# gMedAI-Lab/GAViKO

Measured on AMD Instinct MI355X. Metric: MRI volumes/sec (fwd+bwd) ViT-B/16 gaviko, 120x160x160, higher is better.
Workload: dtype bf16

## Files before the change

### gaviko_amd/csrc/common.hpp

```cpp
#pragma once
#include <hip/hip_runtime.h>
#include <functional>
#include <stdint.h>

namespace gvk {

typedef __bf16 bf16;
typedef __attribute__((ext_vector_type(8))) __bf16 bf16x8;
typedef __attribute__((ext_vector_type(4))) __bf16 bf16x4;
typedef __attribute__((ext_vector_type(2))) __bf16 bf16x2;
typedef __attribute__((ext_vector_type(4))) float f32x4;
typedef __attribute__((ext_vector_type(2))) float f32x2;
typedef __attribute__((ext_vector_type(16))) float f32x16;
typedef __attribute__((ext_vector_type(4))) short s16x4;
typedef __attribute__((ext_vector_type(4))) unsigned int u32x4;
typedef __attribute__((ext_vector_type(2))) unsigned int u32x2;

#define GVK_LDS __attribute__((address_space(3)))
#define GVK_GLOBAL __attribute__((address_space(1)))

constexpr int kWave = 64;

__device__ __forceinline__ int lane_id() { return threadIdx.x & 63; }
__device__ __forceinline__ int wave_id() { return __builtin_amdgcn_readfirstlane(threadIdx.x >> 6); }

__device__ __forceinline__ float wave_sum(float v) {
#pragma unroll
  for (int o = 32; o > 0; o >>= 1) v += __shfl_xor(v, o, 64);
  return v;
}
__device__ __forceinline__ float wave_max(float v) {
#pragma unroll
  for (int o = 32; o > 0; o >>= 1) v = fmaxf(v, __shfl_xor(v, o, 64));
  return v;
}

__device__ __forceinline__ void xcd_group_block(int bid, int nblk, int ngrp, int& grp, int& blk) {
  const int per = ngrp >> 3, main = per * 8 * nblk;
  if (bid < main) {
    const int xcd = bid & 7, j = bid >> 3;
    grp = (j / nblk) * 8 + xcd;
    blk = j - (j / nblk) * nblk;
  } else {
    const int r = bid - main;
    grp = per * 8 + r / nblk;
    blk = r - (r / nblk) * nblk;
  }
}

__device__ __forceinline__ void glds16(const void* gsrc, void* lds_wave_base) {
  __builtin_amdgcn_global_load_lds((const GVK_GLOBAL void*)gsrc, (GVK_LDS void*)lds_wave_base, 16, 0, 0);
}

__device__ __forceinline__ bf16x4 lds_read_tr16(const void* p) {
  s16x4 v = __builtin_amdgcn_ds_read_tr16_b64_v4i16((GVK_LDS s16x4*)p);
  return __builtin_bit_cast(bf16x4, v);
}

__device__ __forceinline__ float as_poly(float t) {
  float p = __builtin_fmaf(t, 1.061405429f, -1.453152027f);
  p = __builtin_fmaf(t, p, 1.421413741f);
  p = __builtin_fmaf(t, p, -0.284496736f);
  p = __builtin_fmaf(t, p, 0.254829592f);
  return t * p;
}
__device__ __forceinline__ float erf_fast(float x) {
  const float ax = fabsf(x);
  const float t = __builtin_amdgcn_rcpf(__builtin_fmaf(0.3275911f, ax, 1.0f));
  const float e = __builtin_amdgcn_exp2f(ax * ax * -1.44269504088896340736f);
  const float r = __builtin_fmaf(-as_poly(t), e, 1.0f);
  return copysignf(r, x);
}
__device__ __forceinline__ float gelu_erf(float x) { return 0.5f * x * (1.0f + erff(x * 0.70710678118654752440f)); }
__device__ __forceinline__ float gelu_erf_grad(float x) {
  return 0.5f * (1.0f + erff(x * 0.70710678118654752440f)) + x * 0.39894228040143267794f * __expf(-0.5f * x * x);
}
__device__ __forceinline__ float gelu_fast(float x) {
  const float h = 0.5f * x;
  return __builtin_fmaf(h, erf_fast(x * 0.70710678118654752440f), h);
}
__device__ __forceinline__ float gelu_fast_grad(float x) {
  const float ax = fabsf(x) * 0.70710678118654752440f;
  const float t = __builtin_amdgcn_rcpf(__builtin_fmaf(0.3275911f, ax, 1.0f));
  const float e = __builtin_amdgcn_exp2f(x * x * -0.72134752044448170368f);
  const float erfv = copysignf(__builtin_fmaf(-as_poly(t), e, 1.0f), x);
  return __builtin_fmaf(x * 0.39894228040143267794f, e, __builtin_fmaf(0.5f, erfv, 0.5f));
}
__device__ __forceinline__ void gelu_fast_both(float x, float& y, float& dy) {
  const float z = x * 0.70710678118654752440f, ax = fabsf(z);
  const float t = __builtin_amdgcn_rcpf(__builtin_fmaf(0.3275911f, ax, 1.0f));
  const float e = __builtin_amdgcn_exp2f(ax * ax * -1.44269504088896340736f);
  const float erfv = copysignf(__builtin_fmaf(-as_poly(t), e, 1.0f), z);
  const float h = 0.5f * x;
  y = __builtin_fmaf(h, erfv, h);
  dy = __builtin_fmaf(x * 0.39894228040143267794f, e, __builtin_fmaf(0.5f, erfv, 0.5f));
}
__device__ __forceinline__ float sigmoidf_(float x) { return 1.0f / (1.0f + __expf(-x)); }
__device__ __forceinline__ float quick_gelu(float x) { return x * sigmoidf_(1.702f * x); }
__device__ __forceinline__ float quick_gelu_grad(float x) {
  float s = sigmoidf_(1.702f * x);
  return s + 1.702f * x * s * (1.0f - s);
}

}

#include <stdlib.h>
namespace gvk {
#ifdef GVK_DIAG
inline const char* diag_env(const char* name) { return getenv(name); }
#else
inline const char* diag_env(const char*) { return nullptr; }
#endif
}

extern "C" const char* gvk_last_error(void);
namespace gvk {
int set_error(int code, const char* fmt, ...);

bool plan_recording();
void plan_push(std::function<void()>&& node);
void plan_push_launch(hipStream_t stream, std::function<void()>&& node);

template <typename... KArgs, typename... Args>
inline void launch(void (*kernel)(KArgs...), dim3 grid, dim3 block, unsigned lds, hipStream_t stream, Args... args) {
  if (plan_recording())
    plan_push_launch(stream, [=]() { hipLaunchKernelGGL(kernel, grid, block, lds, stream, static_cast<KArgs>(args)...); });
  hipLaunchKernelGGL(kernel, grid, block, lds, stream, static_cast<KArgs>(args)...);
}
#define GVK_LAUNCH(kernel, grid, block, lds, stream, ...) ::gvk::launch(kernel, grid, block, lds, stream, __VA_ARGS__)

int check_launch(const char* what);
}

#define GVK_REQUIRE(cond, ...)                                  \
  do {                                                          \
    if (!(cond)) return gvk::set_error(-2, __VA_ARGS__);        \
  } while (0)
```

### gaviko_amd/csrc/runtime.hip

```cpp
#include "common.hpp"
#include "../../include/gaviko_hip.h"
#include <cstdarg>
#include <cstdio>
#include <cstdlib>
#include <cstring>
#include <memory>
#include <mutex>
#include <vector>

namespace gvk {
static thread_local char g_err[512] = "";

int set_error(int code, const char* fmt, ...) {
  va_list ap;
  va_start(ap, fmt);
  vsnprintf(g_err, sizeof(g_err), fmt, ap);
  va_end(ap);
  return code;
}

int check_launch(const char* what) {
  hipError_t e = hipGetLastError();
  if (e != hipSuccess) return set_error(-1, "%s: launch failed: %s", what, hipGetErrorString(e));
  return 0;
}

struct Plan {
  std::vector<std::function<void()>> nodes;
  std::vector<hipEvent_t> events;
  ~Plan() {
    for (hipEvent_t e : events) (void)hipEventDestroy(e);
  }
};
static thread_local Plan* g_rec = nullptr;
static std::mutex g_plans_mu;
static std::vector<std::unique_ptr<Plan>> g_plans;

static bool g_plan_timing = false;
bool plan_recording() { return g_rec != nullptr; }
void plan_push(std::function<void()>&& node) { g_rec->nodes.push_back(std::move(node)); }

#ifdef GVK_DIAG
__global__ void nop_kernel() {}
static std::vector<hipStream_t> g_nop_streams;
void plan_push_launch(hipStream_t stream, std::function<void()>&& node) {
  for (hipStream_t s : g_nop_streams)
    if (s == stream) {
      g_rec->nodes.push_back([=]() { hipLaunchKernelGGL(nop_kernel, dim3(1), dim3(64), 0, stream); });
      return;
    }
  g_rec->nodes.push_back(std::move(node));
}
#else
void plan_push_launch(hipStream_t, std::function<void()>&& node) { g_rec->nodes.push_back(std::move(node)); }
#endif

__global__ void seed_advance_kernel(unsigned long long* seed, unsigned long long inc) { seed[0] += inc; }
__global__ __launch_bounds__(256) void fill_u32_kernel(unsigned* p, unsigned v, long n4, long n) {
  const long stride = (long)gridDim.x * 256;
  for (long i = (long)blockIdx.x * 256 + threadIdx.x; i < n4; i += stride) ((uint4*)p)[i] = uint4{v, v, v, v};
  for (long i = 4 * n4 + (long)blockIdx.x * 256 + threadIdx.x; i < n; i += stride) p[i] = v;
}
__global__ __launch_bounds__(256) void copy_u32_kernel(unsigned* dst, const unsigned* src, long n4, long n) {
  const long stride = (long)gridDim.x * 256;
  for (long i = (long)blockIdx.x * 256 + threadIdx.x; i < n4; i += stride) ((uint4*)dst)[i] = ((const uint4*)src)[i];
  for (long i = 4 * n4 + (long)blockIdx.x * 256 + threadIdx.x; i < n; i += stride) dst[i] = src[i];
}
__global__ void scale_kernel(float* x, float alpha, long n) {
  const long i = (long)blockIdx.x * blockDim.x + threadIdx.x;
  if (i < n) x[i] *= alpha;
}
}

#ifdef GVK_DIAG
extern "C" int gvk_plan_nop_stream(void* stream) {
  gvk::g_nop_streams.push_back((hipStream_t)stream);
  return 0;
}
extern "C" int gvk_plan_nop_clear(void) {
  gvk::g_nop_streams.clear();
  return 0;
}
#endif

extern "C" int gvk_plan_begin(void) {
  using namespace gvk;
  GVK_REQUIRE(g_rec == nullptr, "gvk_plan_begin: a plan is already being recorded on this thread");
  g_rec = new Plan();
  return 0;
}

extern "C" int gvk_plan_abort(void) {
  delete gvk::g_rec;
  gvk::g_rec = nullptr;
  return 0;
}

extern "C" int gvk_plan_end(void) {
  using namespace gvk;
  GVK_REQUIRE(g_rec != nullptr, "gvk_plan_end: no plan is being recorded");
  std::lock_guard<std::mutex> lk(g_plans_mu);
  g_plans.emplace_back(g_rec);
  g_rec = nullptr;
  return (int)g_plans.size() - 1;
}

extern "C" int gvk_plan_size(int plan) {
  using namespace gvk;
  std::lock_guard<std::mutex> lk(g_plans_mu);
  GVK_REQUIRE(plan >= 0 && plan < (int)g_plans.size() && g_plans[plan], "gvk_plan_size: no such plan %d", plan);
  return (int)g_plans[plan]->nodes.size();
}

extern "C" int gvk_plan_replay(int plan) {
  using namespace gvk;
  Plan* p = nullptr;
  {
    std::lock_guard<std::mutex> lk(g_plans_mu);
    GVK_REQUIRE(plan >= 0 && plan < (int)g_plans.size() && g_plans[plan], "gvk_plan_replay: no such plan %d", plan);
    p = g_plans[plan].get();
  }
  GVK_REQUIRE(g_rec == nullptr, "gvk_plan_replay: cannot replay while recording");
  for (auto& node : p->nodes) node();
  return check_launch("plan_replay");
}

extern "C" int gvk_plan_free(int plan) {
  using namespace gvk;
  std::lock_guard<std::mutex> lk(g_plans_mu);
  GVK_REQUIRE(plan >= 0 && plan < (int)g_plans.size() && g_plans[plan], "gvk_plan_free: no such plan %d", plan);
  g_plans[plan].reset();
  return 0;
}

extern "C" int gvk_plan_set_timing(int on) {
  gvk::g_plan_timing = on != 0;
  return 0;
}

extern "C" int gvk_plan_event_elapsed(int plan, int e0, int e1, float* ms) {
  using namespace gvk;
  std::lock_guard<std::mutex> lk(g_plans_mu);
  GVK_REQUIRE(plan >= 0 && plan < (int)g_plans.size() && g_plans[plan], "gvk_plan_event_elapsed: no such plan %d", plan);
  Plan* p = g_plans[plan].get();
  GVK_REQUIRE(e0 >= 0 && e1 >= 0 && e0 < (int)p->events.size() && e1 < (int)p->events.size() && ms, "gvk_plan_event_elapsed: bad event ids");
  hipError_t e = hipEventElapsedTime(ms, p->events[e0], p->events[e1]);
  if (e != hipSuccess) return set_error(-1, "hipEventElapsedTime: %s (timing needs GAVIKO_HIP_PLAN_TIMING=1 at record time)", hipGetErrorString(e));
  return 0;
}

static int plan_event_record_impl(void* stream, bool force_sys_fence);
extern "C" int gvk_plan_event_record(void* stream) { return plan_event_record_impl(stream, false); }
extern "C" int gvk_plan_event_record_fenced(void* stream) { return plan_event_record_impl(stream, true); }

static int plan_event_record_impl(void* stream, bool force_sys_fence) {
  using namespace gvk;
  GVK_REQUIRE(g_rec != nullptr, "gvk_plan_event_record: only valid while a plan is being recorded");
  static const bool env_timing = getenv("GAVIKO_HIP_PLAN_TIMING") != nullptr;
  hipEvent_t ev;
  static const bool sys_fence = diag_env("GAVIKO_HIP_EVENT_FENCE") != nullptr;
  const unsigned flags = ((env_timing || g_plan_timing) ? hipEventDefault : hipEventDisableTiming) | ((sys_fence || force_sys_fence) ? 0u : hipEventDisableSystemFence);
  hipError_t e = hipEventCreateWithFlags(&ev, flags);
  if (e != hipSuccess) return set_error(-1, "hipEventCreate: %s", hipGetErrorString(e));
  g_rec->events.push_back(ev);
  hipStream_t s = (hipStream_t)stream;
  g_rec->nodes.push_back([=]() { (void)hipEventRecord(ev, s); });
  e = hipEventRecord(ev, s);
  if (e != hipSuccess) return set_error(-1, "hipEventRecord: %s", hipGetErrorString(e));
  return (int)g_rec->events.size() - 1;
}

extern "C" int gvk_plan_event_stream_wait(int plan, int event, void* stream) {
  using namespace gvk;
  hipEvent_t ev;
  {
    std::lock_guard<std::mutex> lk(g_plans_mu);
    GVK_REQUIRE(plan >= 0 && plan < (int)g_plans.size() && g_plans[plan], "gvk_plan_event_stream_wait: no such plan %d", plan);
    Plan* p = g_plans[plan].get();
    GVK_REQUIRE(event >= 0 && event < (int)p->events.size(), "gvk_plan_event_stream_wait: no such event %d", event);
    ev = p->events[event];
  }
  hipError_t e = hipStreamWaitEvent((hipStream_t)stream, ev, 0);
  if (e != hipSuccess) return set_error(-1, "hipStreamWaitEvent: %s", hipGetErrorString(e));
  return 0;
}

extern "C" int gvk_plan_event_wait(void* stream, int event) {
  using namespace gvk;
  GVK_REQUIRE(g_rec != nullptr, "gvk_plan_event_wait: only valid while a plan is being recorded");
  GVK_REQUIRE(event >= 0 && event < (int)g_rec->events.size(), "gvk_plan_event_wait: no such event %d", event);
  hipEvent_t ev = g_rec->events[event];
  hipStream_t s = (hipStream_t)stream;
  g_rec->nodes.push_back([=]() { (void)hipStreamWaitEvent(s, ev, 0); });
  hipError_t e = hipStreamWaitEvent(s, ev, 0);
  if (e != hipSuccess) return set_error(-1, "hipStreamWaitEvent: %s", hipGetErrorString(e));
  return 0;
}

extern "C" int gvk_memset_async(void* ptr, int value, size_t bytes, void* stream) {
  using namespace gvk;
  GVK_REQUIRE(ptr != nullptr || bytes == 0, "gvk_memset_async: null pointer");
  if (bytes == 0) return 0;
  GVK_REQUIRE(((uintptr_t)ptr & 15) == 0 && bytes % 4 == 0, "gvk_memset_async: pointer must be 16-byte aligned and the size a multiple of 4");
  const unsigned b = (unsigned)value & 0xFFu, v = b | (b << 8) | (b << 16) | (b << 24);
  const long n = (long)(bytes / 4), n4 = n / 4;
  long blocks = (n4 + 255) / 256;
  blocks = blocks < 1 ? 1 : (blocks > 2048 ? 2048 : blocks);
  GVK_LAUNCH(fill_u32_kernel, dim3((unsigned)blocks), dim3(256), 0, (hipStream_t)stream, (unsigned*)ptr, v, n4, n);
  return check_launch("memset_async");
}

extern "C" int gvk_seed_advance(void* seed, uint64_t inc, void* stream) {
  using namespace gvk;
  GVK_REQUIRE(seed != nullptr, "gvk_seed_advance: null pointer");
  GVK_LAUNCH(seed_advance_kernel, dim3(1), dim3(1), 0, (hipStream_t)stream, (unsigned long long*)seed, (unsigned long long)inc);
  return check_launch("seed_advance");
}

extern "C" int gvk_scale_f32(float* x, float alpha, long n, void* stream) {
  using namespace gvk;
  GVK_REQUIRE(x != nullptr && n >= 0, "gvk_scale_f32: bad arguments");
  if (n == 0) return 0;
  GVK_LAUNCH(scale_kernel, dim3((unsigned)((n + 255) / 256)), dim3(256), 0, (hipStream_t)stream, x, alpha, n);
  return check_launch("scale_f32");
}

extern "C" const char* gvk_last_error(void) { return gvk::g_err; }
extern "C" int gvk_abi_version(void) { return 14; }

extern "C" int gvk_device_check(void) {
  int dev = 0;
  hipError_t e = hipGetDevice(&dev);
  if (e != hipSuccess) return gvk::set_error(-1, "hipGetDevice: %s", hipGetErrorString(e));
  hipDeviceProp_t prop;
  e = hipGetDeviceProperties(&prop, dev);
  if (e != hipSuccess) return gvk::set_error(-1, "hipGetDeviceProperties: %s", hipGetErrorString(e));
  if (strncmp(prop.gcnArchName, "gfx950", 6) != 0)
    return gvk::set_error(-4, "libgaviko_hip is built for gfx950 only; device %d is %s", dev, prop.gcnArchName);
  return 950;
}
```

### gaviko_amd/lib.py

```python
from __future__ import annotations

import ctypes as C
import os

import torch

_HERE = os.path.dirname(os.path.abspath(__file__))
if os.environ.get("GPU_MAX_HW_QUEUES") is None:
    os.environ["GPU_MAX_HW_QUEUES"] = "8"
    try:
        import sys as _sys
        _t = _sys.modules.get("torch")
        if _t is not None and _t.cuda.is_initialized():
            import warnings as _w
            _w.warn("gaviko_amd: HIP was initialised before gaviko_amd was imported, so GPU_MAX_HW_QUEUES=8 cannot take effect; the three "
                    "streams of a step may share hardware queues (slower, not wrong).  Import gaviko_amd first or export the variable.")
    except Exception:
        pass

ABI_VERSION = 14
DIAG = os.environ.get("GAVIKO_HIP_DIAG", "0") == "1"
LIB_PATH = os.environ.get("GAVIKO_HIP_LIB") or os.path.join(_HERE, "libgaviko_hip_diag.so" if DIAG else "libgaviko_hip.so")


def diag_env(name: str, default=None):
    return os.environ.get(name, default) if DIAG else default


class GemmDesc(C.Structure):
    _fields_ = [
        ("a", C.c_void_p), ("w", C.c_void_p), ("out0", C.c_void_p), ("out1", C.c_void_p),
        ("bias", C.c_void_p), ("res", C.c_void_p), ("aux", C.c_void_p), ("pos", C.c_void_p), ("seed_ptr", C.c_void_p),
        ("M", C.c_int32), ("N", C.c_int32), ("K", C.c_int32),
        ("lda", C.c_int32), ("ldw", C.c_int32), ("ldo", C.c_int32), ("ldres", C.c_int32), ("ldaux", C.c_int32),
        ("epilogue", C.c_int32), ("rows_in", C.c_int32), ("rows_out", C.c_int32), ("row_off", C.c_int32),
        ("tile", C.c_int32), ("drop_p", C.c_float), ("seed", C.c_uint64),
        ("scale_cols", C.c_int32), ("col_scale", C.c_float),
        ("ln_mean", C.c_void_p), ("ln_rstd", C.c_void_p), ("ln_c1", C.c_void_p), ("stat_part", C.c_void_p), ("stat_pivot", C.c_void_p),
        ("m_panels", C.c_int32), ("m_stride", C.c_int32), ("splitk_ws", C.c_void_p), ("splitk_ws_bytes", C.c_uint64),
        ("ksplit", C.c_int32), ("aux_is_grad", C.c_int32),
    ]


def _struct(name, ptrs, ints, floats=(), u64=(), i64=()):
    fields = [(f, C.c_void_p) for f in ptrs] + [(f, C.c_int32) for f in ints] + [(f, C.c_float) for f in floats] + \
             [(f, C.c_uint64) for f in u64] + [(f, C.c_int64) for f in i64]
    return type(name, (C.Structure,), {"_fields_": fields})


SkinnyDownDesc = _struct("SkinnyDownDesc",
                         ["x", "w", "bias", "ln_gamma", "ln_beta", "mean", "rstd", "z", "y", "w2", "y2", "seed_ptr"],
                         ["M", "C", "L", "L2", "act", "w_layout", "act_in"], ["eps", "drop_p"], ["seed"])
SkinnyUpDesc = _struct("SkinnyUpDesc", ["lat", "w", "bias", "res", "out", "lat_override", "seed_ptr", "ln_x", "ln_mean", "ln_rstd", "ln_gamma", "out_bf16",
                                        "alpha_ptr", "gg_x", "w2", "bias2", "z2", "y2", "lat_b", "w_b",
                                        "nx_w", "nx_bias", "nx_ln_gamma", "nx_ln_beta", "nx_mean", "nx_rstd", "nx_lat", "nx_w2", "nx_y2"],
                       ["M", "C", "L", "T", "P", "w_layout", "accumulate", "L2", "act2", "w2_layout", "nx_L2"], ["drop_p", "drop2_p", "nx_eps"],
                       ["seed", "seed2"])
OuterDesc = _struct("OuterDesc", ["narrow", "wide", "lat_override", "mean", "rstd", "ln_gamma", "ln_beta", "scratch", "out", "colsum", "seed_ptr",
                                  "narrow2", "wide2"],
                    ["M", "C", "L", "T", "P", "transposed", "accumulate", "wide_act", "M2"], ["drop_p"], ["seed"])
WindowAttnDesc = _struct("WindowAttnDesc", ["qkv", "ctx", "lse", "dctx", "delta", "dqkv", "seed_ptr"],
                         ["B", "D", "H", "W", "kd", "kh", "kw", "L"], ["scale", "drop_p"], ["seed"])
GpaDesc = _struct("GpaDesc",
                  ["xl", "ll", "ca0_g", "ca0_b", "ca1_w", "ca1_b", "ca3_w", "ca3_b", "gl0_g", "gl0_b", "gl1_w", "gl1_b",
                   "wgq", "bgq", "wlq", "blq", "imp", "gw", "enh", "prm", "qg", "ql", "cg", "cl", "lse_g", "lse_l",
                   "dcomb", "zx", "zl", "dimp", "dgw_part", "dqg", "dql", "dcg", "dcl", "delta_g", "delta_l", "dprm",
                   "dcls", "gate_partials", "dzx", "dzl", "enh16"],
                  ["B", "T", "N", "P", "L", "ld16", "col16"], ["scale"])
SsfColgradDesc = _struct("SsfColgradDesc", ["dy", "y0", "y1", "pos", "s", "t", "ds", "dt", "scratch"],
                         ["M", "N", "ld_dy", "ld_y", "dy_f32", "y0_f32", "rows_in", "rows_out", "row_off", "y0_cols"], ["y0_mul", "y_mul"])
DvptDesc = _struct("DvptDesc", ["z", "enh", "lse", "dcomb", "gate", "bu", "colsum_dy", "delta", "dz", "dgate"], ["B", "T", "P", "L", "C"], ["scale"])
AdamDesc = _struct("AdamDesc", ["ptr_tab", "blk_tab", "grad", "m", "v", "norm_sq"], ["nblocks"],
                   ["lr", "beta1", "beta2", "eps", "bias_c1", "bias_c2", "max_norm"])
LossDesc = _struct("LossDesc", ["logits", "target", "weights", "loss", "dlogits", "meter"], ["B", "K", "kind", "reduction"], ["gamma", "eps"], i64=["ignore_index"])
DropoutDesc = _struct("DropoutDesc", ["x", "out32", "out16", "seed_ptr"], ["M", "N", "ld", "rows_in", "rows_out", "row_off"], ["drop_p"], ["seed"])
RowProjDesc = _struct("RowProjDesc", ["w", "bias", "y", "z", "y_split"], ["L", "w_layout", "act", "ld_split", "col_split"])
LnBwdDesc = _struct("LnBwdDesc", ["dy", "x", "mean", "rstd", "gamma", "dres", "dx", "dx_bf16", "proj"],
                    ["M", "C", "groups", "rows_per_group", "group_stride", "dy_bf16"])
AttentionDesc = _struct("AttentionDesc", ["qkv", "out", "lse", "dout", "delta", "dqkv", "seed_ptr", "ws"],
                        ["B", "T", "H", "ld_qkv", "ld_out", "f32", "need_rows"], ["scale", "drop_p"], ["seed", "ws_bytes"])
ReduceJob = _struct("ReduceJob", ["a", "b", "out", "a2"], ["M", "J", "L", "accumulate", "M2"])
PgradOuter = _struct("PgradOuter", ["narrow", "wide", "narrow2", "wide2", "lat_override", "mean", "rstd", "out", "colsum",
                                    "aff_w", "aff_gamma", "aff_beta", "aff_dgamma", "aff_dbeta", "aff_dbias"],
                     ["M", "M2", "T", "P", "transposed", "accumulate", "C"], ["drop_p"], ["seed"])
WindowColsumDesc = _struct("WindowColsumDesc", ["qkv", "lse", "w", "out"], ["B", "D", "H", "W", "kd", "kh", "kw", "L"], ["scale"])
GpaMapsDesc = _struct("GpaMapsDesc", ["xl", "ll", "qg", "ql", "lse_g", "lse_l", "imp", "gw", "pg", "pl", "fused"], ["B", "T", "N", "P", "L"])
FeatureTopkDesc = _struct("FeatureTopkDesc", ["q", "g", "exclude", "idx", "score", "scratch"], ["Nq", "Ng", "C", "k", "metric", "nslabs"],
                          i64=["scratch_words"])
HeadDesc = _struct("HeadDesc", ["g", "ln_gamma", "ln_beta", "wh", "bh", "logits", "pooled", "dlogits", "dg", "dwh", "dbh"],
                   ["B", "T", "C", "K", "r0", "R", "accumulate"])

(EPI_STORE_BF16, EPI_BIAS_RES_F32, EPI_BIAS_GELU_BF16, EPI_PATCH_F32, EPI_GELU_BWD_BF16, EPI_STORE_F32, EPI_BIAS_RES_F32_BF16,
 EPI_BIAS_RELU_BF16, EPI_RELU_BWD_BF16) = range(9)

_P, _I, _F, _L = C.c_void_p, C.c_int, C.c_float, C.c_int64
SIGNATURES = {
    "gvk_gemm_nt_bf16": [C.POINTER(GemmDesc), _P],
    "gvk_gemm_nt_f32": [C.POINTER(GemmDesc), _P],
    "gvk_patchify_f32": [_P, _P, _I, _I, _I, _I, _I, _I, _I, _P],
    "gvk_transpose_f32": [_P, _P, _I, _I, _P],
    "gvk_transpose_bf16": [_P, _P, _I, _I, _P],
    "gvk_copy_async": [_P, _P, C.c_size_t, _P],
    "gvk_copy_f32_strided": [_P, _P, _I, _I, _I, _P],
    "gvk_cast_f32_bf16": [_P, _P, _L, _P],
    "gvk_transpose_cast_f32_bf16": [_P, _P, _I, _I, _P],
    "gvk_pack_split_bf16": [_P, _I, _P, _P, _I, _I, _I, _I, _P],
    "gvk_prompt_up_fix": [_P, _P, _P, _P, _I, _I, _I, _I, _I, _P],
    "gvk_layernorm_fwd_fix": [_P, _P, _P, _P, _P, _P, _I, _I, _F, _P, _P, _P, _I, _I, _I, _P],
    "gvk_patchify_bf16": [_P, _P, _I, _I, _I, _I, _I, _I, _I, _P],
    "gvk_layernorm_fwd": [_P, _P, _P, _P, _P, _P, _P, _I, _I, _F, _P],
    "gvk_layernorm_bwd": [C.POINTER(LnBwdDesc), _P],
    "gvk_layernorm_bwd_affine": [_P, _P, _P, _P, _P, _P, _P, _I, _I, _I, _P],
    "gvk_attention_fwd": [C.POINTER(AttentionDesc), _P],
    "gvk_attention_bwd": [C.POINTER(AttentionDesc), _P],
    "gvk_qkv_prescale_bf16": [_P, _I, _I, _I, _F, _P],
    "gvk_prompt_up_fix_stats": [_P, _P, _P, _P, _P, _P, _I, _P, _P, _P, _I, _I, _I, _I, _I, _F, _P],
    "gvk_attention_colsum_bf16": [_P, _P, _P, _I, _P, _I, _I, _I, _I, _I, _I, _P],
    "gvk_rollout_step": [_P, _P, _P, _I, _I, _I, _P],
    "gvk_attention_gradcolsum_bf16": [_P, _P, _P, _I, _P, _I, _P, _I, _I, _I, _I, _I, _I, _P],
    "gvk_relevance_step": [_P, _P, _P, _I, _I, _I, _P],
    "gvk_unpatchify_f32": [_P, _P, _P, _P, _I, _I, _I, _I, _I, _I, _I, _I, _F, _F, _P],
    "gvk_patch_reduce_f32": [_P, _P, _I, _I, _I, _I, _I, _I, _I, _I, _P],
    "gvk_evp_highpass_sign": [_P, _P, _P, _P, _P, _I, _I, _I, _I, _P],
    "gvk_evp_highpass_linear": [_P, _P, _P, _P, _I, _I, _I, _I, _I, _P],
    "gvk_skinny_down": [C.POINTER(SkinnyDownDesc), _P],
    "gvk_skinny_up": [C.POINTER(SkinnyUpDesc), _P],
    "gvk_outer_reduce": [C.POINTER(OuterDesc), _P],
    "gvk_small_wgrad": [_P, _P, _P, _P, _I, _I, _I, _I, _P],
    "gvk_ln_lowrank_affine": [_P, _P, _P, _P, _P, _P, _P, _P, _P, _I, _I, _I, _P],
    "gvk_colsum": [_P, _P, _P, _I, _I, _I, _P],
    "gvk_reduce_batch": [C.POINTER(ReduceJob), _I, _P, _P],
    "gvk_param_grads": [C.POINTER(PgradOuter), _I, C.POINTER(ReduceJob), _I, _P, _L, _P, _I, _P, _I, _I, _P],
    "gvk_window_attn_fwd": [C.POINTER(WindowAttnDesc), _P],
    "gvk_window_attn_bwd": [C.POINTER(WindowAttnDesc), _P],
    "gvk_gpa_fwd": [C.POINTER(GpaDesc), _P],
    "gvk_gpa_bwd": [C.POINTER(GpaDesc), _P],
    "gvk_window_attn_colsum": [C.POINTER(WindowColsumDesc), _P],
    "gvk_gpa_attn_maps": [C.POINTER(GpaMapsDesc), _P],
    "gvk_rows_broadcast": [_P, _P, _P, _I, _I, _I, _I, _I, _P],
    "gvk_rows_batch_sum": [_P, _P, _P, _I, _I, _I, _I, _I, _I, _P],
    "gvk_small_linear_fwd": [_P, _P, _P, _P, _I, _I, _I, _P],
    "gvk_small_linear_bwd": [_P, _P, _P, _P, _P, _P, _I, _I, _I, _I, _P],
    "gvk_vpt_repack_fwd": [_P, _P, _P, _I, _I, _I, _I, _I, _I, _P],
    "gvk_vpt_repack_bwd": [_P, _P, _I, _I, _I, _I, _I, _I, _P],
    "gvk_cast_bf16_f32_strided": [_P, _P, _I, _I, _I, _P],
    "gvk_lora_merge_f32": [_P, _P, _P, _P, _P, _P, _I, _I, _F, _P],
    "gvk_layernorm_fwd_proj": [_P, _P, _P, _P, _P, _P, _I, _I, _F, C.POINTER(RowProjDesc), _P],
    "gvk_layernorm_bwd_up": [_P, _P, _P, _P, _P, _P, _P, _P, _P, _P, _I, _I, _I, _I, _P],
    "gvk_ssf_fold_weight": [_P, _P, _P, _P, _I, _I, _I, _P],
    "gvk_ssf_fold_vec": [_P, _P, _P, _P, _I, _P],
    "gvk_ssf_colgrad": [C.POINTER(SsfColgradDesc), _P],
    "gvk_ssf_ln_grad": [_P, _P, _P, _P, _P, _P, _I, _P],
    "gvk_ssf_head_grad": [_P, _P, _P, _P, _P, _P, _P, _P, _P, _I, _I, _I, _I, _I, _I, _P],
    "gvk_dvpt_fwd": [C.POINTER(DvptDesc), _P],
    "gvk_dvpt_bwd": [C.POINTER(DvptDesc), _P],
    "gvk_scale_dev": [_P, _P, C.c_int64, _P],
    "gvk_evp_highpass": [_P, _P, _P, _P, _I, _I, _I, _I, _P],
    "gvk_pad2d_f32": [_P, _I, _I, _I, _I, _P, _I, _I, _I, _P],
    "gvk_add2d_f32": [_P, _I, _P, _I, _P, _I, _I, _I, _P],
    "gvk_gelu_fwd_f32": [_P, _P, C.c_int64, _P],
    "gvk_gelu_bwd_f32": [_P, _P, _P, C.c_int64, _P],
    "gvk_rows_patch": [_P, _P, _P, _I, _I, _I, _I, _I, _I, _P],
    "gvk_rows_gather": [_P, _P, _I, _I, _I, _I, _I, _P],
    "gvk_sumsq": [_P, C.c_int64, _P, _P, _P],
    "gvk_adam_step": [C.POINTER(AdamDesc), _P],
    "gvk_loss_fwd_bwd": [C.POINTER(LossDesc), _P],
    "gvk_dropout_rows": [C.POINTER(DropoutDesc), _P],
    "gvk_volume_minmax": [_P, _P, _I, _L, _P],
    "gvk_rescale_intensity": [_P, _P, _P, _P, _I, _L, _F, _F, _P],
    "gvk_spatial_transform": [_P, _P, _P, _P, _P, _I, _I, _I, _I, _P],
    "gvk_gaussian_blur3d": [_P, _P, _P, _P, _P, _I, _I, _I, _I, _I, _P],
    "gvk_intensity_pointwise": [_P, _P, _P, _P, _P, _P, _I, _I, _I, _I, _I, _P],
    "gvk_motion_artifact": [_P, _P, _P, _P, _P, _P, _I, _I, _I, _I, _I, _P],
    "gvk_eval_rows": [_P, _P, _P, _P, _P, _I, _I, _P],
    "gvk_ovr_auc_counts": [_P, _P, _P, _I, _I, _P],
    "gvk_memset_async": [_P, _I, C.c_size_t, _P],
    "gvk_seed_advance": [_P, C.c_uint64, _P],
    "gvk_scale_f32": [_P, _F, C.c_long, _P],
    "gvk_head_fwd": [C.POINTER(HeadDesc), _P],
    "gvk_head_bwd": [C.POINTER(HeadDesc), _P],
    "gvk_patch_rank": [_P, _P, _I, _I, _P],
    "gvk_patch_mask_rank": [_P, _P, _P, _P, _P, _I, _I, _I, _P],
    "gvk_patch_mask_box": [_P, _P, _I, _I, _I, _I, _P],
    "gvk_perturb_volume": [_P, _P, _P, _P, _P, _I, _P, _I, _I, _I, _I, _I, _I, _I, _I, _P],
    "gvk_perturb_scores": [_P, _P, _P, _P, _P, _P, _P, _I, _I, _I, _I, _P],
    "gvk_curve_auc": [_P, _P, _P, _I, _I, _I, _P],
    "gvk_tta_volumes": [_P, _P, _P, _P, _I, _I, _I, _I, _I, _P],
    "gvk_predictive_stats": [_P, _P, _P, _P, _P, _P, _P, _P, _P, _I, _I, _I, _P],
    "gvk_calibration_bins": [_P, _P, _P, _P, _P, _P, _P, _I, _I, _I, _P],
    "gvk_token_pool": [_P, _P, _I, _I, _I, _I, _I, _P],
    "gvk_l2_normalize_rows": [_P, _P, _P, _I, _I, _F, _P],
    "gvk_feature_topk": [C.POINTER(FeatureTopkDesc), _P],
    "gvk_knn_vote": [_P, _P, _P, _P, _P, _I, _I, _I, _I, _I, _F, _P],
    "gvk_class_means": [_P, _P, _P, _P, _I, _I, _I, _P],
}
NO_STREAM = {"gvk_last_error": (C.c_char_p, []), "gvk_device_check": (C.c_int, []), "gvk_abi_version": (C.c_int, []),
             "gvk_attention_bwd_ws_bytes": (C.c_size_t, [C.c_int, C.c_int, C.c_int]),
             "gvk_attention_bwd_status_offset": (C.c_size_t, [C.c_size_t]),
             "gvk_gpa_gate_param_count": (C.c_int, [C.c_int, C.c_int]), "gvk_gemm_stat_parts": (C.c_int, [C.c_int]), "gvk_minmax_partials": (C.c_int, []),
             "gvk_param_grads_scratch": (C.c_int64, [C.POINTER(PgradOuter), C.c_int, C.POINTER(ReduceJob), C.c_int, C.c_int, C.c_int]),
             "gvk_feature_topk_slabs": (C.c_int, [C.c_int, C.c_int, C.c_int]),
             "gvk_plan_begin": (C.c_int, []), "gvk_plan_end": (C.c_int, []), "gvk_plan_abort": (C.c_int, []),
             "gvk_plan_size": (C.c_int, [C.c_int]), "gvk_plan_replay": (C.c_int, [C.c_int]), "gvk_plan_free": (C.c_int, [C.c_int]),
             "gvk_plan_event_record": (C.c_int, [_P]), "gvk_plan_event_wait": (C.c_int, [_P, C.c_int]),
             "gvk_plan_event_record_fenced": (C.c_int, [_P]), "gvk_plan_event_stream_wait": (C.c_int, [C.c_int, C.c_int, _P]),
             "gvk_plan_set_timing": (C.c_int, [C.c_int]),
             "gvk_plan_event_elapsed": (C.c_int, [C.c_int, C.c_int, C.c_int, C.POINTER(C.c_float)])}
STRUCTS = {"gvk_gemm_desc": GemmDesc, "gvk_skinny_down_desc": SkinnyDownDesc, "gvk_skinny_up_desc": SkinnyUpDesc,
           "gvk_outer_desc": OuterDesc, "gvk_window_attn_desc": WindowAttnDesc, "gvk_gpa_desc": GpaDesc, "gvk_window_colsum_desc": WindowColsumDesc, "gvk_gpa_maps_desc": GpaMapsDesc, "gvk_head_desc": HeadDesc, "gvk_reduce_job": ReduceJob, "gvk_pgrad_outer": PgradOuter, "gvk_rowproj_desc": RowProjDesc, "gvk_attention_desc": AttentionDesc, "gvk_adam_desc": AdamDesc, "gvk_loss_desc": LossDesc, "gvk_dropout_desc": DropoutDesc, "gvk_ssf_colgrad_desc": SsfColgradDesc, "gvk_dvpt_desc": DvptDesc,
           "gvk_feature_topk_desc": FeatureTopkDesc}

DIAG_SIGNATURES = {}
DIAG_NO_STREAM = {"gvk_plan_nop_stream": (C.c_int, [_P]), "gvk_plan_nop_clear": (C.c_int, [])}

_lib = None


class GavikoHipError(RuntimeError):
    pass


def load() -> C.CDLL:
    global _lib
    if _lib is not None:
        return _lib
    if not os.path.exists(LIB_PATH):
        raise GavikoHipError(
            f"{LIB_PATH} not found: build it with `python -m gaviko_amd.build` (hipcc, gfx950). "
            "gaviko_amd has no CPU or eager fallback.")
    lib = C.CDLL(LIB_PATH)
    for name, (res, args) in NO_STREAM.items():
        fn = getattr(lib, name)
        fn.restype, fn.argtypes = res, args
    for name, args in SIGNATURES.items():
        fn = getattr(lib, name)
        fn.restype, fn.argtypes = C.c_int, args
    if DIAG:
        for name, (res, args) in DIAG_NO_STREAM.items():
            fn = getattr(lib, name)
            fn.restype, fn.argtypes = res, args
        for name, args in DIAG_SIGNATURES.items():
            fn = getattr(lib, name)
            fn.restype, fn.argtypes = C.c_int, args
    if lib.gvk_abi_version() != ABI_VERSION:
        raise GavikoHipError(f"{LIB_PATH} has ABI version {lib.gvk_abi_version()}, these bindings describe {ABI_VERSION}: rebuild with "
                             "`python -m gaviko_amd.build`")
    _lib = lib
    return lib


def check(rc: int, what: str) -> None:
    if rc != 0:
        raise GavikoHipError(f"{what} failed (rc={rc}): {load().gvk_last_error().decode()}")


_device_ok = False


def require_device() -> None:
    global _device_ok
    if _device_ok:
        return
    if not torch.cuda.is_available():
        raise GavikoHipError("no HIP device visible: gaviko_amd runs on MI355X (gfx950) only and has no CPU fallback")
    rc = load().gvk_device_check()
    if rc != 950:
        raise GavikoHipError(f"gvk_device_check: {load().gvk_last_error().decode()}")
    _device_ok = True


def stream_ptr() -> int:
    return torch.cuda.current_stream().cuda_stream


def ptr(t) -> int:
    return 0 if t is None else t.data_ptr()
```

### include/gaviko_hip_diag.h

```cpp
#ifndef GAVIKO_HIP_DIAG_H
#define GAVIKO_HIP_DIAG_H
#include "gaviko_hip.h"
#ifdef __cplusplus
extern "C" {
#endif

int gvk_plan_nop_stream(void* stream);
int gvk_plan_nop_clear(void);

#ifdef __cplusplus
}
#endif
#endif
```

Measured before the change: 768.6.

## Reduce replayed plan sync edges: attach events to launches, merge records, drop implied waits

```diff
diff --git a/gaviko_amd/csrc/common.hpp b/gaviko_amd/csrc/common.hpp
--- a/gaviko_amd/csrc/common.hpp
+++ b/gaviko_amd/csrc/common.hpp
@@ -1,5 +1,6 @@
 #pragma once
 #include <hip/hip_runtime.h>
+#include <hip/hip_ext.h>
 #include <functional>
 #include <stdint.h>
 
@@ -118,13 +119,19 @@
 int set_error(int code, const char* fmt, ...);
 
 bool plan_recording();
-void plan_push(std::function<void()>&& node);
-void plan_push_launch(hipStream_t stream, std::function<void()>&& node);
+void plan_push_launch(hipStream_t stream, std::function<void(hipEvent_t)>&& node);
 
 template <typename... KArgs, typename... Args>
 inline void launch(void (*kernel)(KArgs...), dim3 grid, dim3 block, unsigned lds, hipStream_t stream, Args... args) {
-  if (plan_recording())
-    plan_push_launch(stream, [=]() { hipLaunchKernelGGL(kernel, grid, block, lds, stream, static_cast<KArgs>(args)...); });
+  if (plan_recording()) {
+    plan_push_launch(stream, [=](hipEvent_t stop) {
+      if (stop)
+        hipExtLaunchKernelGGL(kernel, grid, block, lds, stream, nullptr, stop, 0u, static_cast<KArgs>(args)...);
+      else
+        hipLaunchKernelGGL(kernel, grid, block, lds, stream, static_cast<KArgs>(args)...);
+    });
+    return;
+  }
   hipLaunchKernelGGL(kernel, grid, block, lds, stream, static_cast<KArgs>(args)...);
 }
 #define GVK_LAUNCH(kernel, grid, block, lds, stream, ...) ::gvk::launch(kernel, grid, block, lds, stream, __VA_ARGS__)
diff --git a/gaviko_amd/csrc/plan_reduce.hpp b/gaviko_amd/csrc/plan_reduce.hpp
--- /dev/null
+++ b/gaviko_amd/csrc/plan_reduce.hpp
@@ -0,0 +1,74 @@
+#pragma once
+#include <algorithm>
+#include <vector>
+
+namespace gvk {
+
+struct PlanOp {
+  enum Kind { LAUNCH, RECORD, WAIT } kind;
+  const void* stream;
+  int event;
+  bool mergeable;
+};
+
+struct PlanReduction {
+  std::vector<char> keep;
+  std::vector<int> alias;
+  int merged = 0, implied = 0;
+};
+
+inline PlanReduction plan_reduce(const std::vector<PlanOp>& ops, int n_events) {
+  PlanReduction r;
+  r.keep.assign(ops.size(), 1);
+  r.alias.resize(n_events);
+  for (int i = 0; i < n_events; ++i) r.alias[i] = i;
+
+  std::vector<const void*> streams;
+  auto sid = [&](const void* s) {
+    for (size_t i = 0; i < streams.size(); ++i)
+      if (streams[i] == s) return (int)i;
+    streams.push_back(s);
+    return (int)streams.size() - 1;
+  };
+  for (const PlanOp& op : ops) (void)sid(op.stream);
+  const int S = (int)streams.size();
+
+  std::vector<int> last(S, -1);
+  std::vector<int> pos(S, 0);
+  std::vector<std::vector<int>> known(S, std::vector<int>(S, 0));
+  std::vector<std::vector<int>> clock(n_events);
+
+  for (size_t i = 0; i < ops.size(); ++i) {
+    const PlanOp& op = ops[i];
+    const int s = sid(op.stream);
+    ++pos[s];
+    known[s][s] = pos[s];
+    const bool records = (op.kind == PlanOp::RECORD || op.kind == PlanOp::LAUNCH) && op.event >= 0 && op.event < n_events;
+    if (records) clock[op.event] = known[s];
+    if (op.kind == PlanOp::RECORD && records && op.mergeable && last[s] >= 0) {
+      const PlanOp& prev = ops[last[s]];
+      const bool prev_records = (prev.kind == PlanOp::RECORD || prev.kind == PlanOp::LAUNCH) && prev.event >= 0;
+      if (prev_records && prev.mergeable) {
+        r.alias[op.event] = r.alias[prev.event];
+        r.keep[i] = 0;
+        ++r.merged;
+        continue;
+      }
+    }
+    if (op.kind == PlanOp::WAIT && op.event >= 0 && op.event < n_events && !clock[op.event].empty()) {
+      const std::vector<int>& c = clock[op.event];
+      bool covered = true;
+      for (int b = 0; b < S; ++b) covered = covered && c[b] <= known[s][b];
+      if (covered) {
+        r.keep[i] = 0;
+        ++r.implied;
+        continue;
+      }
+      for (int b = 0; b < S; ++b) known[s][b] = std::max(known[s][b], c[b]);
+    }
+    last[s] = (int)i;
+  }
+  return r;
+}
+
+}
diff --git a/gaviko_amd/csrc/runtime.hip b/gaviko_amd/csrc/runtime.hip
--- a/gaviko_amd/csrc/runtime.hip
+++ b/gaviko_amd/csrc/runtime.hip
@@ -1,4 +1,5 @@
 #include "common.hpp"
+#include "plan_reduce.hpp"
 #include "../../include/gaviko_hip.h"
 #include <cstdarg>
 #include <cstdio>
@@ -25,11 +26,30 @@
   return 0;
 }
 
+struct Node {
+  PlanOp::Kind kind;
+  hipStream_t stream;
+  int event;
+  std::function<void(hipEvent_t)> launch;
+};
 struct Plan {
-  std::vector<std::function<void()>> nodes;
+  std::vector<Node> nodes;
   std::vector<hipEvent_t> events;
+  std::vector<char> mergeable;
+  std::vector<hipEvent_t> owned;
+  int merged = 0, implied = 0;
   ~Plan() {
-    for (hipEvent_t e : events) (void)hipEventDestroy(e);
+    for (hipEvent_t e : owned) (void)hipEventDestroy(e);
+  }
+  void run() {
+    for (Node& n : nodes) {
+      if (n.kind == PlanOp::LAUNCH)
+        n.launch(n.event >= 0 ? events[n.event] : nullptr);
+      else if (n.kind == PlanOp::RECORD)
+        (void)hipEventRecord(events[n.event], n.stream);
+      else
+        (void)hipStreamWaitEvent(n.stream, events[n.event], 0);
+    }
   }
 };
 static thread_local Plan* g_rec = nullptr;
@@ -38,21 +58,25 @@
 
 static bool g_plan_timing = false;
 bool plan_recording() { return g_rec != nullptr; }
-void plan_push(std::function<void()>&& node) { g_rec->nodes.push_back(std::move(node)); }
 
 #ifdef GVK_DIAG
 __global__ void nop_kernel() {}
 static std::vector<hipStream_t> g_nop_streams;
-void plan_push_launch(hipStream_t stream, std::function<void()>&& node) {
+void plan_push_launch(hipStream_t stream, std::function<void(hipEvent_t)>&& node) {
   for (hipStream_t s : g_nop_streams)
     if (s == stream) {
-      g_rec->nodes.push_back([=]() { hipLaunchKernelGGL(nop_kernel, dim3(1), dim3(64), 0, stream); });
+      g_rec->nodes.push_back(Node{PlanOp::LAUNCH, stream, -1, [=](hipEvent_t stop) {
+        if (stop) hipExtLaunchKernelGGL(nop_kernel, dim3(1), dim3(64), 0, stream, nullptr, stop, 0u);
+        else hipLaunchKernelGGL(nop_kernel, dim3(1), dim3(64), 0, stream);
+      }});
       return;
     }
-  g_rec->nodes.push_back(std::move(node));
+  g_rec->nodes.push_back(Node{PlanOp::LAUNCH, stream, -1, std::move(node)});
 }
 #else
-void plan_push_launch(hipStream_t, std::function<void()>&& node) { g_rec->nodes.push_back(std::move(node)); }
+void plan_push_launch(hipStream_t stream, std::function<void(hipEvent_t)>&& node) {
+  g_rec->nodes.push_back(Node{PlanOp::LAUNCH, stream, -1, std::move(node)});
+}
 #endif
 
 __global__ void seed_advance_kernel(unsigned long long* seed, unsigned long long inc) { seed[0] += inc; }
@@ -81,6 +105,25 @@
   gvk::g_nop_streams.clear();
   return 0;
 }
+extern "C" int gvk_plan_edge_counts(int plan, void* stream, int* out) {
+  using namespace gvk;
+  std::lock_guard<std::mutex> lk(g_plans_mu);
+  GVK_REQUIRE(plan >= 0 && plan < (int)g_plans.size() && g_plans[plan] && out, "gvk_plan_edge_counts: no such plan %d", plan);
+  for (int i = 0; i < 10; ++i) out[i] = 0;
+  for (const Node& n : g_plans[plan]->nodes)
+    for (int base = 0; base <= 4; base += 4) {
+      if (base == 4 && n.stream != (hipStream_t)stream) continue;
+      if (n.kind == PlanOp::LAUNCH) {
+        ++out[base];
+        if (n.event >= 0) ++out[base + 1];
+      } else {
+        ++out[base + (n.kind == PlanOp::RECORD ? 2 : 3)];
+      }
+    }
+  out[8] = g_plans[plan]->merged;
+  out[9] = g_plans[plan]->implied;
+  return 0;
+}
 #endif
 
 extern "C" int gvk_plan_begin(void) {
@@ -99,10 +142,28 @@
 extern "C" int gvk_plan_end(void) {
   using namespace gvk;
   GVK_REQUIRE(g_rec != nullptr, "gvk_plan_end: no plan is being recorded");
-  std::lock_guard<std::mutex> lk(g_plans_mu);
-  g_plans.emplace_back(g_rec);
+  Plan* p = g_rec;
   g_rec = nullptr;
-  return (int)g_plans.size() - 1;
+  static const bool no_reduce = diag_env("GAVIKO_HIP_EDGE_REDUCE") != nullptr && diag_env("GAVIKO_HIP_EDGE_REDUCE")[0] == '0';
+  if (!no_reduce) {
+    std::vector<PlanOp> ops;
+    ops.reserve(p->nodes.size());
+    for (const Node& n : p->nodes) ops.push_back(PlanOp{n.kind, (const void*)n.stream, n.event, n.kind != PlanOp::WAIT && n.event >= 0 && p->mergeable[n.event] != 0});
+    const PlanReduction r = plan_reduce(ops, (int)p->events.size());
+    std::vector<Node> kept;
+    kept.reserve(p->nodes.size());
+    for (size_t i = 0; i < p->nodes.size(); ++i)
+      if (r.keep[i]) kept.push_back(std::move(p->nodes[i]));
+    p->nodes.swap(kept);
+    p->merged = r.merged;
+    p->implied = r.implied;
+    for (size_t e = 0; e < p->events.size(); ++e) p->events[e] = p->events[r.alias[e]];
+  }
+  p->run();
+  int rc = check_launch("plan_end");
+  std::lock_guard<std::mutex> lk(g_plans_mu);
+  g_plans.emplace_back(p);
+  return rc != 0 ? rc : (int)g_plans.size() - 1;
 }
 
 extern "C" int gvk_plan_size(int plan) {
@@ -121,7 +182,7 @@
     p = g_plans[plan].get();
   }
   GVK_REQUIRE(g_rec == nullptr, "gvk_plan_replay: cannot replay while recording");
-  for (auto& node : p->nodes) node();
+  p->run();
   return check_launch("plan_replay");
 }
 
@@ -162,12 +223,25 @@
   const unsigned flags = ((env_timing || g_plan_timing) ? hipEventDefault : hipEventDisableTiming) | ((sys_fence || force_sys_fence) ? 0u : hipEventDisableSystemFence);
   hipError_t e = hipEventCreateWithFlags(&ev, flags);
   if (e != hipSuccess) return set_error(-1, "hipEventCreate: %s", hipGetErrorString(e));
+  const bool plain = flags == (hipEventDisableTiming | hipEventDisableSystemFence);
   g_rec->events.push_back(ev);
+  g_rec->owned.push_back(ev);
+  g_rec->mergeable.push_back(plain ? 1 : 0);
+  const int idx = (int)g_rec->events.size() - 1;
   hipStream_t s = (hipStream_t)stream;
-  g_rec->nodes.push_back([=]() { (void)hipEventRecord(ev, s); });
-  e = hipEventRecord(ev, s);
-  if (e != hipSuccess) return set_error(-1, "hipEventRecord: %s", hipGetErrorString(e));
-  return (int)g_rec->events.size() - 1;
+  static const bool no_attach = diag_env("GAVIKO_HIP_EDGE_ATTACH") != nullptr && diag_env("GAVIKO_HIP_EDGE_ATTACH")[0] == '0';
+  if (plain && !no_attach)
+    for (size_t i = g_rec->nodes.size(); i-- > 0;) {
+      Node& n = g_rec->nodes[i];
+      if (n.stream != s) continue;
+      if (n.kind == PlanOp::LAUNCH && n.event < 0) {
+        n.event = idx;
+        return idx;
+      }
+      break;
+    }
+  g_rec->nodes.push_back(Node{PlanOp::RECORD, s, idx, nullptr});
+  return idx;
 }
 
 extern "C" int gvk_plan_event_stream_wait(int plan, int event, void* stream) {
@@ -189,11 +263,7 @@
   using namespace gvk;
   GVK_REQUIRE(g_rec != nullptr, "gvk_plan_event_wait: only valid while a plan is being recorded");
   GVK_REQUIRE(event >= 0 && event < (int)g_rec->events.size(), "gvk_plan_event_wait: no such event %d", event);
-  hipEvent_t ev = g_rec->events[event];
-  hipStream_t s = (hipStream_t)stream;
-  g_rec->nodes.push_back([=]() { (void)hipStreamWaitEvent(s, ev, 0); });
-  hipError_t e = hipStreamWaitEvent(s, ev, 0);
-  if (e != hipSuccess) return set_error(-1, "hipStreamWaitEvent: %s", hipGetErrorString(e));
+  g_rec->nodes.push_back(gvk::Node{PlanOp::WAIT, (hipStream_t)stream, event, nullptr});
   return 0;
 }
 
diff --git a/gaviko_amd/lib.py b/gaviko_amd/lib.py
--- a/gaviko_amd/lib.py
+++ b/gaviko_amd/lib.py
@@ -211,7 +211,8 @@
            "gvk_feature_topk_desc": FeatureTopkDesc}
 
 DIAG_SIGNATURES = {}
-DIAG_NO_STREAM = {"gvk_plan_nop_stream": (C.c_int, [_P]), "gvk_plan_nop_clear": (C.c_int, [])}
+DIAG_NO_STREAM = {"gvk_plan_nop_stream": (C.c_int, [_P]), "gvk_plan_nop_clear": (C.c_int, []),
+                  "gvk_plan_edge_counts": (C.c_int, [C.c_int, _P, C.POINTER(C.c_int)])}
 
 _lib = None
 
diff --git a/include/gaviko_hip_diag.h b/include/gaviko_hip_diag.h
--- a/include/gaviko_hip_diag.h
+++ b/include/gaviko_hip_diag.h
@@ -7,6 +7,7 @@
 
 int gvk_plan_nop_stream(void* stream);
 int gvk_plan_nop_clear(void);
+int gvk_plan_edge_counts(int plan, void* stream, int* out);
 
 #ifdef __cplusplus
 }
```

Result: no change. 765.5 (-0.4%).
